# Gepetto/mpc-interface

Hardware: AMD Instinct MI355X
Metric: QP assemblies/sec (P,q,G,h), biped N=16 batched (higher is better)
Workload: dtype f64; 1 GPU; C2 biped LIPM N=16 no=36 nc=76, per-instance (A,B)/given/aim, K1 on chip; batch_per_gpu=4096, global_batch=4096, streams=2

## Files before the change

include/mpcasm.h:

```cpp
#ifndef MPCASM_H
#define MPCASM_H

#include <stddef.h>
#include <stdint.h>

#ifdef __cplusplus
extern "C" {
#endif

typedef enum mpcasm_status {
  MPCASM_OK = 0,
  MPCASM_ERR_ARG = -1,
  MPCASM_ERR_PLAN = -2,
  MPCASM_ERR_HIP = -3,
  MPCASM_ERR_NODEVICE = -4,
  MPCASM_ERR_LIMIT = -5
} mpcasm_status;

typedef struct mpcasm_plan mpcasm_plan;


int mpcasm_abi_version(void);
int mpcasm_device_count(void);
int mpcasm_last_hip(void);
const char* mpcasm_status_string(int status);
enum { MPCASM_OPT_PATH = 1, MPCASM_OPT_PHASE_MASK = 2, MPCASM_OPT_RESIDENT_PER_CU = 3, MPCASM_OPT_JIT = 4,
       MPCASM_OPT_P_DIRECT = 5, MPCASM_OPT_RESIDENT_GRID = 6 };
int mpcasm_set_option(int option, int value);
int mpcasm_plan_set_option(mpcasm_plan* plan, int option, int value);
int mpcasm_resident_lds_bytes(const int32_t* h_itab, size_t n_itab, const double* h_dtab, size_t n_dtab,
                              int64_t out[2]);
int mpcasm_jit_check(const int32_t* h_itab, size_t n_itab, const double* h_dtab, size_t n_dtab,
                     char* log, size_t log_capacity);

int mpcasm_plan_prepare(const mpcasm_plan* plan, int batch);
int mpcasm_jit_stats(int64_t out[3]);

int mpcasm_fill_su(const double* d_A, const double* d_B, double* d_S, double* d_U,
                   int batch, int N, int n, int m, int ltv, void* stream);

int mpcasm_plan_create(const int32_t* h_itab, size_t n_itab,
                       const double* h_dtab, size_t n_dtab,
                       mpcasm_plan** out_plan);
int mpcasm_plan_destroy(mpcasm_plan* plan);

int mpcasm_plan_sizes(const mpcasm_plan* plan, int64_t out[8]);

int mpcasm_plan_csc_sizes(const mpcasm_plan* plan, int64_t out[2]);
// ... 99 lines not shown
```

mpc-interface_amd/csrc/capi.hip:

```cpp
#include <hip/hip_runtime.h>
#include <stdint.h>
#include <stdlib.h>
#include <string.h>

#include <algorithm>
#include <cmath>
#include <mutex>
#include <new>
#include <string>
#include <vector>

#include "jit.h"
#include "kernels.h"

using namespace mpcasm;

namespace mpcasm {
int g_p_direct = 0;
extern int g_path;
extern int g_phase_mask;
extern int g_resident_per_cu, g_resident_grid;
}

struct mpcasm_plan {
// ... 1055 lines not shown
  if (option == MPCASM_OPT_P_DIRECT) {
    if (value < 0 || value > 2) return MPCASM_ERR_ARG;
    g_p_direct = value;
    return MPCASM_OK;
  }
  if (option == MPCASM_OPT_JIT) {
    if (value < 0 || value > 2) return MPCASM_ERR_ARG;
    g_jit = value;
    return MPCASM_OK;
  }
  if (option == MPCASM_OPT_RESIDENT_PER_CU) {
    if (value < 0 || value > 16) return MPCASM_ERR_ARG;
    g_resident_per_cu = value;
    return MPCASM_OK;
  }
  if (option == MPCASM_OPT_RESIDENT_GRID) {
    if (value < 0 || value > (1 << 20)) return MPCASM_ERR_ARG;
    g_resident_grid = value;
    return MPCASM_OK;
  }
  return MPCASM_ERR_ARG;
}

int mpcasm_plan_set_option(mpcasm_plan* plan, int option, int value) {
  if (!plan) return MPCASM_ERR_ARG;
  if (option == MPCASM_OPT_PATH && value >= -1 && value <= 4) plan->opt_path = value;
  else if (option == MPCASM_OPT_JIT && value >= -1 && value <= 2) plan->opt_jit = value;
  else if (option == MPCASM_OPT_RESIDENT_PER_CU && value >= -1 && value <= 16) plan->opt_per_cu = value;
  else if (option == MPCASM_OPT_RESIDENT_GRID && value >= -1 && value <= (1 << 20)) plan->opt_grid = value;
  else return MPCASM_ERR_ARG;
// ... 102 lines not shown
  PlanDev d;
  memset(&d, 0, sizeof d);
  plan_dev_from_tables(h_itab, &d);
  if (!d.rs_ok) return MPCASM_ERR_LIMIT;
  std::vector<char> code;
  std::string text;
  const int small = resident_p_direct_for(d, 1), large = resident_p_direct_for(d, 1 << 30);
  int out = MPCASM_OK;
  if (!jit_available()) {
    text = "libhiprtc.so could not be loaded";
    out = MPCASM_ERR_LIMIT;
  } else {
    for (int form : {small, large}) {
      if (form == large && small != large && out != MPCASM_OK) break;
      d.rs_p_direct = form;
      out = jit_code_for(jit_spec_header(d, h_itab), false, 0xBF, &code, &text) ? MPCASM_OK : MPCASM_ERR_HIP;
      if (small == large) break;
    }
  }
  if (log && log_capacity) {
    strncpy(log, text.c_str(), log_capacity - 1);
    log[log_capacity - 1] = 0;
  }
  return out;
}

int mpcasm_jit_stats(int64_t out[3]) {
  if (!out) return MPCASM_ERR_ARG;
  long v[3];
  jit_stats(v);
  out[0] = v[0];
  out[1] = v[1];
  out[2] = v[2];
  return MPCASM_OK;
}

int mpcasm_plan_prepare(const mpcasm_plan* plan, int batch) {
  if (!plan || batch < 0) return MPCASM_ERR_ARG;
  int current = -1;
// ... 460 lines not shown
```

mpc-interface_amd/csrc/jit.h:

```cpp
#pragma once
#include <hip/hip_runtime.h>
#include <stdint.h>

#include <string>
#include <vector>

#include "plan_dev.h"

namespace mpcasm {

extern int g_jit;
extern int g_phase_mask;

std::string jit_spec_header(const PlanDev& d, const int32_t* h_itab);
int jit_compile(const std::string& header, std::vector<char>* code, std::string* log,
                bool stamps = false, int phases = 0xBF);
const void* jit_kernel_for(const PlanDev& d, const int32_t* h_itab, int device, int batch,
                           size_t lds_bytes);
bool jit_code_for(const std::string& header, bool stamps, int phases, std::vector<char>* code,
                  std::string* log, bool distrust_disk = false);
bool jit_available();
void jit_stats(long out[3]);
void jit_forget(const void* itab);
int jit_launch(const void* kernel, const PlanDev& p, const SrcTable& src, const double* params,
               const double* given, double* P, double* q, double* G, double* h, int batch,
               int num_cus, int per_cu_limit, int grid_limit, void* work, hipStream_t stream, hipError_t* err);

}
```

mpc-interface_amd/csrc/jit.hip:

```cpp
#include <dlfcn.h>
#include <hip/hip_runtime.h>
#include <stdint.h>
#include <stdio.h>
#include <stdlib.h>
#include <string.h>

#include <sys/stat.h>
#include <sys/types.h>
#include <unistd.h>

#include <atomic>
#include <condition_variable>
#include <iterator>
#include <map>
#include <mutex>
#include <string>
#include <vector>

#include "jit.h"
#include "kernels.h"

namespace mpcasm {

int g_jit = 0;

namespace {

#include "jit_embed.inc"

constexpr int JIT_MIN_BATCH = 512;

struct Rtc {
  typedef struct _hiprtcProgram* Program;
  int (*create)(Program*, const char*, const char*, int, const char* const*, const char* const*);
  int (*compile)(Program, int, const char* const*);
  int (*log_size)(Program, size_t*);
  int (*get_log)(Program, char*);
  int (*code_size)(Program, size_t*);
  int (*get_code)(Program, char*);
// ... 20 lines not shown
    r.get_code = reinterpret_cast<decltype(r.get_code)>(sym("hiprtcGetCode"));
    r.destroy = reinterpret_cast<decltype(r.destroy)>(sym("hiprtcDestroyProgram"));
    r.ok = r.create && r.compile && r.log_size && r.get_log && r.code_size && r.get_code && r.destroy;
  });
  return r;
}

void append(std::string& s, const char* fmt, long long v) {
  char buf[96];
  snprintf(buf, sizeof buf, fmt, v);
  s += buf;
}

}

std::string jit_spec_header(const PlanDev& d, const int32_t* it) {
  std::string s = "// generated by libmpcasm (jit.hip) for one plan\n#pragma once\n"
                  "namespace mpcasm {\nnamespace spec {\nstruct PlanConst {\n";
#define MPCASM_X(f) append(s, "  static constexpr int " #f " = %lld;\n", (long long)d.f);
  MPCASM_PLAN_INT_FIELDS(MPCASM_X)
#undef MPCASM_X
  append(s, "  static constexpr unsigned rs_src16 = %lldu;\n};\n", (long long)d.rs_src16);
  const int jc = d.rs_jc <= 3 ? 3 : d.rs_jc <= 4 ? 4 : d.rs_jc <= 5 ? 5 : d.rs_jc <= 8 ? 8 : RS_JC_MAX;
  append(s, "constexpr int JC = %lld;\n", jc);
  append(s, "constexpr int NTRIP = %lld;\n", d.rs_ntrip);
  s += "constexpr int TRIPS[NTRIP + 1][8] = {\n";
  const int32_t* tr = it + d.off_rs_trip;
  for (int t = 0; t <= d.rs_ntrip; ++t) {
    s += "  {";
    for (int k = 0; k < RS_TRIP_WORDS; ++k) append(s, k ? ", %lld" : "%lld", tr[t * RS_TRIP_WORDS + k]);
    s += "},\n";
  }
  s += "};\nconstexpr int WTRIP[8][2] = {";
  const int32_t* wt = it + d.off_rs_wtrip;
  for (int w = 0; w < RS_WAVES; ++w) {
    append(s, "{%lld, ", wt[2 * w]);
    append(s, "%lld}, ", wt[2 * w + 1]);
  }
  s += "};\n}  // namespace spec\n}  // namespace mpcasm\n";
  return s;
}

int jit_compile(const std::string& header, std::vector<char>* code, std::string* log, bool stamps,
                int phases) {
  const Rtc& r = rtc();
  if (!r.ok) {
    if (log) *log = "libhiprtc.so could not be loaded";
    return MPCASM_ERR_LIMIT;
  }
  const char* headers[] = {header.c_str(), k_src_device_prims, k_src_plan_dev, k_src_plan_tables};
  const char* names[] = {"plan_spec.h", "device_prims.h", "plan_dev.h", "plan_tables.h"};
  Rtc::Program prog = nullptr;
// ... 110 lines not shown

struct JitKernel {
  hipModule_t module = nullptr;
  hipFunction_t fn = nullptr;
  int per_cu = 0;
  size_t lds = 0;
  bool failed = false;
  bool building = true;
};

std::mutex g_mutex;
std::condition_variable g_built;
std::map<std::pair<int, std::string>, JitKernel*> g_cache;
struct FastKey {
  const void* itab;
  int device, p_direct, phases;
  bool operator<(const FastKey& o) const {
    if (itab != o.itab) return itab < o.itab;
    if (device != o.device) return device < o.device;
    if (p_direct != o.p_direct) return p_direct < o.p_direct;
    return phases < o.phases;
  }
};
std::map<FastKey, JitKernel*> g_fast;

}

bool jit_code_for(const std::string& header, bool stamps, int phases, std::vector<char>* code,
                  std::string* log_out, bool distrust_disk) {
  const char* waves = getenv("MPCASM_JIT_WAVES_PER_EU");
  const std::string options = std::string(stamps ? "stamps " : "") + "phases " + std::to_string(phases) +
                              " waves " + (waves ? waves : "4") +
// ... 15 lines not shown
  }
  ++g_stat_compiled;
  if (getenv("MPCASM_JIT_VERBOSE")) fprintf(stderr, "mpcasm: jit: compiled (%zu bytes)\n", code->size());
  if (!path.empty()) disk_write(path, *code);
  return true;
}

namespace {
}

const void* jit_kernel_for(const PlanDev& d, const int32_t* h_itab, int device, int batch,
                           size_t lds_bytes) {
  if (t_jit == 2) return nullptr;
  const bool stamps = (g_phase_mask & 64) != 0;
  const int phases = stamps ? -1 : g_phase_mask;
  const FastKey fast{d.itab, stamps ? device + 4096 : device, d.rs_p_direct, phases};
  const bool may_build = t_jit == 1 || batch >= JIT_MIN_BATCH;
  JitKernel* slot = nullptr;
  bool mine = false;
  std::string header;
  {
    std::unique_lock<std::mutex> lock(g_mutex);
    auto found = g_fast.find(fast);
    if (found != g_fast.end()) {
      slot = found->second;
    } else if (may_build) {
      header = jit_spec_header(d, h_itab);
      JitKernel*& by_text = g_cache[std::make_pair(fast.device, header + "//" + std::to_string(phases))];
      if (by_text == nullptr) {
        by_text = new JitKernel();
        mine = true;
      }
      slot = by_text;
      g_fast[fast] = slot;
    } else {
      return nullptr;
    }
    if (!mine) {
      if (slot->building && !may_build) return nullptr;
      g_built.wait(lock, [&] { return !slot->building; });
    }
  }
// ... 93 lines not shown
```

mpc-interface_amd/csrc/plan_tables.h:

```cpp
#pragma once
#ifndef __HIPCC_RTC__
#include <stdint.h>
#endif

namespace mpcasm {

constexpr int32_t PLAN_MAGIC = 0x4D504341;
constexpr int32_t PLAN_VERSION = 30;

enum HeaderWord : int {
  H_MAGIC = 0,
  H_VERSION,
  H_NG,
  H_NO,
  H_NC,
  H_NPARAMS,
  H_NSRC,
  H_NBASE,
  H_NSEG,
  H_RTOT,
  H_NENT,
  H_NGTERM,
  H_NLIMIT,
  H_NLAX,
// ... 168 lines not shown
enum { GT_AOFF = 0, GT_BOFF, GT_NROWS, GT_WPARAM, GT_DOFF, GT_AIMPARAM, GT_FLAGS, GT_MASKA, GT_MASKB, GT_PAD, GT_WORDS = 10 };
enum { GT_FLAG_P = 1, GT_FLAG_HALF = 2, GT_FLAG_DIAG = 4 };

enum {
  LM_OUT0 = 0, LM_NROWS, LM_NAXES, LM_LAX0,
  LM_ARROW_P, LM_ARROW_ROWS, LM_CENTER_P, LM_CENTER_ROWS, LM_EXTREME_P, LM_EXTREME_ROWS,
  LM_PAD0, LM_PAD1, LM_WORDS = 12
};
enum { LX_ROWOFF = 0, LX_ROWS, LX_WORDS = 2 };

constexpr int MAX_SOURCES = 32;
constexpr int RS_NW = 4, RS_NT = 512, RS_WAVES = RS_NT / 64, RS_JC_MAX = 12, RS_TRIP_WORDS = 8;
constexpr int RS_BLOCKS_MAX = 255;
enum { LT_N = 0, LT_M, LT_HORIZON, LT_A, LT_B, LT_TA, LT_TB, LT_TP, RS_LTI_WORDS = 8 };
constexpr int RS_LTI_MAX = 4;
constexpr int RS_AXMAX = 4, RS_RR_WORDS = 16;
constexpr int RS_GDESC_PIECES = 6, RS_GDESC_THREADS = RS_NT - RS_NW * 64;
constexpr int RS_GFIX_NONE = 7;
constexpr int32_t RS_DST_ACC = 1 << 30;
enum { RT_A = 0, RT_B, RT_D, RT_W, RT_AIM, RT_WORD, RT_BI, RT_BJ };
enum { RT_SHORT = 5, RT_HALF = 6, RT_NOP = 7, RT_FIRST = 8, RT_LAST = 9, RT_LIVE = 10, RT_QMASK = 14,
       RT_TERM_END = 18 };
constexpr int RS_DIAG_MAX = 2;
enum { RR_VOFF = 0, RR_ARROW = 4, RR_CENTER = 8, RR_NAXES = 12, RR_EXTREME = 13, RR_PACKED = 14 };

}
```

mpc-interface_amd/csrc/resident.hip:

```cpp
#ifdef __HIPCC_RTC__
using __hip_internal::int32_t;
using __hip_internal::int64_t;
using __hip_internal::uint32_t;
using __hip_internal::uint64_t;
typedef unsigned long uintptr_t;
#else
#include <hip/hip_runtime.h>
#include <stdint.h>
#endif

#include "device_prims.h"
#include "plan_dev.h"
#ifdef MPCASM_SPEC
#include "plan_spec.h"
#endif
#ifndef __HIPCC_RTC__
#include "kernels.h"
#endif

namespace mpcasm {

#ifndef __HIPCC_RTC__
extern int g_phase_mask;
extern int g_resident_per_cu;
// ... 169 lines not shown
    int lk_ = s.lk, lx_ = s.lx;
    asm volatile("" : "+v"(lk_), "+v"(lx_));
    const int row = 4 * s.bi + lk_, col = 4 * s.bj + lx_;
    if (s.live && row < PC::no) {
      if (s.isq) {
        if (lx_ == 0) s.ql[row] = s.acc + s.dvec[ldp + row];
      } else if (col < PC::no) {
        const double val = s.acc + (row == col ? s.dvec[col] : 0.0);
        s.Pl[row * s.ldpl + col] = val;
        if (PC::rs_sym && s.bi != s.bj) s.Pl[col * s.ldpl + row] = val;
      }
    }
  }
}

template <int I, int N>
__device__ __forceinline__ void spec_trips(TripState& s) {
  if constexpr (I < N) {
    spec_trip<I>(s);
    __builtin_amdgcn_sched_barrier(0);
    spec_trips<I + 1, N>(s);
  }
}
template <int WAVE>
__device__ __forceinline__ void spec_wave_trips(TripState& s) {
  spec_trips<spec::WTRIP[WAVE][0], spec::WTRIP[WAVE][0] + spec::WTRIP[WAVE][1]>(s);
}
#endif

template <int JC, bool STAMPS, bool GEN, class PlanT>
// ... 42 lines not shown
  const int unit = p.rs_unit, nchunk = p.rs_nchunk;
  const int lx = lane & 3, lg = (lane >> 2) & 3, lk = lane >> 4;
  const unsigned ab_lds = (unsigned)(uintptr_t)(lds + L.ab);
  auto fetch_ab = [&](long inst, int slot) {
    for (int k = 0; k < p.rs_ab / 32; ++k) {
      const int2 m = abmeta[k * 64 + lane];
      const char* base = reinterpret_cast<const char* const*>(strm)[2 * m.x];
      const long long stride = reinterpret_cast<const long long*>(strm)[2 * m.x + 1];
      dma4(base + inst * stride + m.y,
           __builtin_amdgcn_readfirstlane(ab_lds + (unsigned)((slot * p.rs_ab + k * 32) * 8)));
    }
  };
  auto generate_sources = [&](int buf, int slot) {
    double* im = lds + L.img + buf * p.rs_img;
    const double* ab = lds + L.ab + slot * p.rs_ab;
    for (int g = 0; g < p.rs_nlti; ++g) {
      const int* rec = lti + g * RS_LTI_WORDS;
      const int n = __builtin_amdgcn_readfirstlane(rec[LT_N]), m = __builtin_amdgcn_readfirstlane(rec[LT_M]);
      const int N = __builtin_amdgcn_readfirstlane(rec[LT_HORIZON]), nn = n * n, nm = n * m;
      const double* Am = ab + __builtin_amdgcn_readfirstlane(rec[LT_A]);
      const double* Bm = ab + __builtin_amdgcn_readfirstlane(rec[LT_B]);
      double* TA = im + __builtin_amdgcn_readfirstlane(rec[LT_TA]);
      double* TB = im + __builtin_amdgcn_readfirstlane(rec[LT_TB]);
      double* TP = im + __builtin_amdgcn_readfirstlane(rec[LT_TP]);
      if (n <= 4 && n + m <= 4) {
        const int grp = lane >> 4, gi = lane & 3, gc = (lane >> 2) & 3;
        const bool live = gi < n && gc < n + m;
        double ar[4];
#pragma unroll
        for (int t = 0; t < 4; ++t) ar[t] = gi < n && t < n ? Am[gi * n + t] : 0.0;
        double x = !live ? 0.0 : (gc < m ? Bm[gi * m + gc] : Am[gi * n + (gc - m)]);
        double* out = gc < m ? TB + gi * m + gc : TA + gi * n + (gc - m);
        const int step = gc < m ? nm : nn;
        auto advance = [&]() {
          double y = ar[0] * quad_broadcast<0>(x);
          y = fma(ar[1], quad_broadcast<1>(x), y);
          y = fma(ar[2], quad_broadcast<2>(x), y);
          y = fma(ar[3], quad_broadcast<3>(x), y);
          x = y;
        };
        const int head = N < 4 ? N : 4;
        for (int d = 0; d < head; ++d) {
          if (live && grp == 0) out[d * step] = x;
          advance();
        }
        if (N > 4) {
          asm volatile("s_waitcnt lgkmcnt(0)" ::: "memory");
#pragma unroll
          for (int t = 0; t < 4; ++t) ar[t] = gi < n && t < n ? TA[3 * nn + gi * n + t] : 0.0;
          x = live ? out[grp * step] : 0.0;
          for (int d = grp + 4; d - grp < N; d += 4) {
            advance();
            if (live && d < N) out[d * step] = x;
          }
        }
        continue;
      }
      for (int e = lane; e < nn; e += 64) {
        const double v = Am[e];
        TA[e] = v;
        TP[e] = v;
      }
      for (int e = lane; e < nm; e += 64) TB[e] = Bm[e];
      asm volatile("s_waitcnt lgkmcnt(0)" ::: "memory");
      int have = 1;
      for (int s_ = 0; have < N; ++s_) {
        const double* Pw = TP + s_ * nn;
        const int cnt = have < N - have ? have : N - have;
        const int na = cnt * nn, nb = cnt * nm, total = na + nb + nn;
        for (int e = lane; e < total; e += 64) {
          const double* X;
// ... 7 lines not shown
            const int d = (e - na) / nm;
            r = (e - na) - d * nm;
            X = TB + d * nm, out = TB + (have + d) * nm, w = m;
          } else {
            r = e - na - nb;
            X = Pw, out = TP + (s_ + 1) * nn, w = n;
          }
          const int i = r / w, j = r - i * w;
          double acc = 0.0;
          for (int t = 0; t < n; ++t) acc = fma(Pw[i * n + t], X[t * w + j], acc);
          out[r] = acc;
        }
        asm volatile("s_waitcnt lgkmcnt(0)" ::: "memory");
        have += cnt;
      }
    }
  };
  const int run_over = (phases >> 10) & 7;
  const int run_shift = run_over ? run_over : ((long)batch >= 16L * gridDim.x && !(phases & 256) ? 2 : 0);
  const unsigned vblock = (phases & 8192) && gridDim.x % 8 == 0
                              ? (blockIdx.x % 8) * (gridDim.x / 8) + blockIdx.x / 8 : blockIdx.x;
  auto instance_at = [&](int n) -> long {
    return ((((long)(n >> run_shift) * gridDim.x + vblock)) << run_shift) + (n & ((1 << run_shift) - 1));
  };
  const bool gen = GEN && p.rs_nlti != 0;
  const int ct = tid - 64, CT = NT - 64;
#ifdef MPCASM_SPEC
  constexpr int ZK = 2;
#else
  constexpr int ZK = 0;
#endif
// ... 72 lines not shown
    for (int k = kfirst; k < nchunk; k += MW) {
      const int2 m = meta[k * 64 + lane];
      const char* base = reinterpret_cast<const char* const*>(strm)[2 * m.x];
      const long long stride = reinterpret_cast<const long long*>(strm)[2 * m.x + 1];
      if (settled && __all(stride == 0)) continue;
      const char* a = base + (m.x == p.nsrc ? ginst : inst) * stride + m.y;
      const unsigned dst = __builtin_amdgcn_readfirstlane(dst0 + (unsigned)(k * 64 * unit));
      if (unit == 16)
        dma16(a, dst);
      else
        dma4(a, dst);
    }
  };
  if (wave == 0) {
    constexpr int MK = 2;
    const int nab2 = p.rs_ab * 2, nmeta = nchunk * 64, nltw = p.rs_nlti * RS_LTI_WORDS;
    const int2* t_ab = reinterpret_cast<const int2*>(plan_itab + p.off_rs_abmeta);
    const int2* t_meta = reinterpret_cast<const int2*>(plan_itab + p.off_rs_inmeta);
    const int32_t* t_lti = plan_itab + p.off_rs_lti;
    int2 v_ab = int2{0, 0}, v_meta[MK];
    int v_lti = 0;
    if (lane < nab2) v_ab = t_ab[lane];
    if (lane < nltw) v_lti = t_lti[lane];
#pragma unroll
    for (int k = 0; k < MK; ++k) v_meta[k] = lane + k * 64 < nmeta ? t_meta[lane + k * 64] : int2{0, 0};
    if (prog_early) load_program();
    if (lane < nab2) abmeta[lane] = v_ab;
    for (int i = lane + 64; i < nab2; i += 64) abmeta[i] = t_ab[i];
    if (lane < nltw) lti[lane] = v_lti;
    for (int i = lane + 64; i < nltw; i += 64) lti[i] = t_lti[i];
#pragma unroll
    for (int k = 0; k < MK; ++k)
      if (lane + k * 64 < nmeta) meta[lane + k * 64] = v_meta[k];
    for (int i = lane + MK * 64; i < nmeta; i += 64) meta[i] = t_meta[i];
    for (int t = 0; t < p.nsrc + 3; ++t) {
      const int s = t - p.nsrc;
      const double* base = s < 0 ? src.ptr[t]
                                 : (s == 0 ? given : (s == 1 ? params : plan_dtab + p.doff_rs_const));
      const long long stride =
          s < 0 ? src.stride[t] : (s == 0 ? (long long)p.ng : (s == 1 ? (long long)p.nparams : 0));
      if (lane == 0) {
        reinterpret_cast<const double**>(strm)[2 * t] = base;
        reinterpret_cast<long long*>(strm)[2 * t + 1] = stride * (long long)sizeof(double);
      }
    }
    if (gen) {
      fetch_ab(instance_at(0), 0);
      if (instance_at(1) < batch) fetch_ab(instance_at(1), 1);
    }
    SETUP_STAMP(2)
    {
      const long inst = instance_at(0), ginst = gix != nullptr ? (long)gix[inst] : inst;
      for (int k = 0; k < nchunk; ++k) {
        const int2 m = meta[k * 64 + lane];
        const char* base = reinterpret_cast<const char* const*>(strm)[2 * m.x];
        const long long stride = reinterpret_cast<const long long*>(strm)[2 * m.x + 1];
        const char* a = base + (m.x == p.nsrc ? ginst : inst) * stride + m.y;
        const unsigned dst = __builtin_amdgcn_readfirstlane(img_lds + (unsigned)(k * 64 * unit));
        if (unit == 16)
          dma16(a, dst);
        else
          dma4(a, dst);
      }
    }
    SETUP_STAMP(0)
    lds_barrier();
    SETUP_STAMP(1)
    prepare_fetch();
    SETUP_STAMP(3)
    if (gen) {
      dma_wait_but(nchunk);
      SETUP_STAMP(4)
      generate_sources(0, 0);
    }
    if (!prog_early) load_program();
    SETUP_STAMP(5)
  } else {
    SETUP_STAMP(0)
    lds_barrier();
    SETUP_STAMP(1)
    prepare_fetch();
    SETUP_STAMP(2)
    load_program();
    typedef int i32x4 __attribute__((ext_vector_type(4)));
    typedef int i32x2 __attribute__((ext_vector_type(2)));
    typedef double f64x2 __attribute__((ext_vector_type(2)));
// ... 712 lines not shown
```

mpc-interface_amd/mpcasm/capi.py:

```python
import ctypes
import os

_HERE = os.path.dirname(os.path.abspath(__file__))
LIB_PATH = os.environ.get("MPCASM_LIB") or os.path.join(_HERE, "libmpcasm.so")

OK = 0
ERR_LIMIT = -5
OPT_PATH = 1
OPT_PHASE_MASK = 2
OPT_RESIDENT_PER_CU = 3
OPT_RESIDENT_GRID = 6
OPT_P_DIRECT = 5
OPT_JIT = 4
PHASE_DEFAULT = 0xBF
PHASE_STAMPS = 0x40
STATUS = {
    0: "MPCASM_OK",
    -1: "MPCASM_ERR_ARG",
    -2: "MPCASM_ERR_PLAN",
    -3: "MPCASM_ERR_HIP",
    -4: "MPCASM_ERR_NODEVICE",
    -5: "MPCASM_ERR_LIMIT",
}
QP_SOLVED, QP_MAX_ITER, QP_PRIMAL_INFEASIBLE, QP_DUAL_INFEASIBLE, QP_NON_CVX = 1, -2, -3, -4, -7
QP_STATUS = {
    1: "MPCASM_QP_SOLVED",
    -2: "MPCASM_QP_MAX_ITER",
# ... 13 lines not shown
    "mpcasm_abi_version": (ctypes.c_int, []),
    "mpcasm_device_count": (ctypes.c_int, []),
    "mpcasm_last_hip": (ctypes.c_int, []),
    "mpcasm_status_string": (ctypes.c_char_p, [ctypes.c_int]),
    "mpcasm_set_option": (ctypes.c_int, [ctypes.c_int, ctypes.c_int]),
    "mpcasm_fill_su": (ctypes.c_int, [_void_p, _void_p, _void_p, _void_p, ctypes.c_int,
                                      ctypes.c_int, ctypes.c_int, ctypes.c_int, ctypes.c_int,
                                      _void_p]),
    "mpcasm_plan_create": (ctypes.c_int, [_void_p, ctypes.c_size_t, _void_p, ctypes.c_size_t,
                                          ctypes.POINTER(_void_p)]),
    "mpcasm_plan_destroy": (ctypes.c_int, [_void_p]),
    "mpcasm_resident_lds_bytes": (ctypes.c_int, [_void_p, ctypes.c_size_t, _void_p, ctypes.c_size_t,
                                                 ctypes.POINTER(ctypes.c_int64)]),
    "mpcasm_jit_check": (ctypes.c_int, [_void_p, ctypes.c_size_t, _void_p, ctypes.c_size_t,
                                        ctypes.c_char_p, ctypes.c_size_t]),
    "mpcasm_plan_sizes": (ctypes.c_int, [_void_p, ctypes.POINTER(ctypes.c_int64)]),
    "mpcasm_plan_csc_sizes": (ctypes.c_int, [_void_p, ctypes.POINTER(ctypes.c_int64)]),
    "mpcasm_plan_set_option": (ctypes.c_int, [_void_p, ctypes.c_int, ctypes.c_int]),
    "mpcasm_assemble_indexed": (ctypes.c_int, [_void_p, ctypes.POINTER(_void_p),
                                               ctypes.POINTER(ctypes.c_int64), _void_p, _void_p, _void_p,
                                               _void_p, _void_p, _void_p, _void_p, _void_p, ctypes.c_int,
                                               _void_p]),
    "mpcasm_plan_last_kernel": (ctypes.c_int, [_void_p]),
    "mpcasm_plan_prepare": (ctypes.c_int, [_void_p, ctypes.c_int]),
    "mpcasm_jit_stats": (ctypes.c_int, [ctypes.POINTER(ctypes.c_int64)]),
    "mpcasm_workspace_bytes": (ctypes.c_int, [_void_p, ctypes.c_int,
                                              ctypes.POINTER(ctypes.c_size_t)]),
    "mpcasm_assemble": (ctypes.c_int, [_void_p, ctypes.POINTER(_void_p),
                                       ctypes.POINTER(ctypes.c_int64), _void_p, _void_p, _void_p,
                                       _void_p, _void_p, _void_p, _void_p, ctypes.c_int, _void_p]),
# ... 89 lines not shown
```

mpc-interface_amd/mpcasm/plan.py:

```python
import collections
import hashlib
from types import SimpleNamespace

import numpy as np
import scipy.sparse as sp

PLAN_MAGIC = 0x4D504341
PLAN_VERSION = 30

_H = {name: i for i, name in enumerate([
    "MAGIC", "VERSION", "NG", "NO", "NC", "NPARAMS", "NSRC", "NBASE", "NSEG", "RTOT", "NENT",
    "NGTERM", "NLIMIT", "NLAX", "PMROWS", "PM_NENT", "LDV",
    "OFF_SEG", "OFF_COLSEG", "OFF_ROWPTR", "OFF_ENTBASE", "OFF_ENTK", "OFF_GTERM", "OFF_LIMIT",
    "OFF_LAX", "OFF_ROWLIMIT", "OFF_PM_ROWPTR", "OFF_PM_ENTBASE", "OFF_PM_ENTK",
    "DOFF_ENTCOEF", "DOFF_PM_ENTCOEF", "NITAB", "NDTAB",
    "FUSED_OK", "ARENA_TOTAL", "OFF_ARENA", "NFD", "OFF_FD_IDX", "OFF_FD_PTR", "NOPS", "OFF_OP",
    "NCOEF", "DOFF_COEFPOOL",
    "RS_OK", "RS_JC", "RS_SYM", "RS_NTRIP", "OFF_RS_SRC", "OFF_RS_GIDX", "OFF_RS_DST",
    "DOFF_RS_COEF", "OFF_RS_TRIP", "OFF_RS_WTRIP", "RS_NSPLIT", "OFF_RS_SPLIT",
    "OFF_RS_RR", "RS_UNIT", "RS_NCHUNK", "OFF_RS_INMETA", "RS_IMG", "RS_IMG_GIVEN",
    "RS_IMG_PARAMS", "DOFF_RS_CONST", "DOFF_DIAGCOEF", "NDIAGCOEF", "RS_NLTI", "OFF_RS_LTI",
    "RS_IMG_DMA", "RS_AB", "OFF_RS_ABMETA", "RR_PACKED", "OFF_RS_DPAR", "DOFF_RS_DCOEF",
    "RS_NGDESC", "OFF_RS_GDESC", "PM_NFD", "OFF_PM_MAP", "OFF_PM_FDPTR", "OFF_PM_OP", "PM_NOPS",
    "DOFF_PM_POOL", "PM_NPOOL", "RS_NZBLK", "OFF_RS_ZBLK", "RS_GSINGLE",
# ... 8 lines not shown
    "SW_OK", "SW_N", "SW_M", "SW_HORIZON", "SW_SRC_A", "SW_SRC_B", "SW_NAXES", "OFF_SW_AXIS", "SW_NTERM",
    "OFF_SW_TERM", "SW_NLIM", "OFF_SW_LIM", "OFF_SW_COL", "SW_DOFF_CVEC", "SW_NCVEC",
    "OFF_SW_CPTR", "OFF_SW_CENT", "SW_NCENT", "OFF_SW_GPTR", "OFF_SW_GENT", "SW_NGENT",
    "OFF_RS_PROG", "T_SCAN_FUSED",
])}
H_WORDS = 160
assert len(_H) <= H_WORDS
RS_NW, RS_NT = 4, 512
RS_WAVES = RS_NT // 64
RS_BLOCKS_MAX = 255
RS_LTI_WORDS, RS_LTI_MAX = 8, 4
RS_JC_MAX = 12
RS_TRIP_WORDS = 8
TRIP_COST, TRIP_STEP_COST, TERM_COST, TRIP_Q_COST, PACK_COST, G_PIECE_COST = 200, 30, 60, 60, 250, 500
G_DESC_PIECE_COST = 330
TABLES_COST, STREAM_WAVE_COST, FETCH_CHUNK_COST = 3300, 500, 350
import os as _os
if _os.environ.get("MPCASM_TRIP_COSTS"):
    _c = [int(x) for x in _os.environ["MPCASM_TRIP_COSTS"].split(",")]
    TRIP_COST, TRIP_STEP_COST, TERM_COST, TRIP_Q_COST, PACK_COST, G_PIECE_COST = _c[:6]
    G_DESC_PIECE_COST = G_PIECE_COST
    if len(_c) > 6:
        TABLES_COST, STREAM_WAVE_COST, FETCH_CHUNK_COST = _c[6:9]
RT_A, RT_B, RT_D, RT_W, RT_AIM, RT_WORD, RT_BI, RT_BJ = range(8)
RT_SHORT, RT_HALF, RT_NOP, RT_FIRST, RT_LAST, RT_LIVE, RT_QMASK, RT_TERM_END = 5, 6, 7, 8, 9, 10, 14, 18
RS_DIAG_MAX = 2
RS_AXMAX = 4
RS_DST_ACC = 1 << 30
RS_GDESC_PIECES, RS_GDESC_THREADS = 6, 256
RS_GFIX_NONE = 7
RS_COMPACT_FROM_BYTES = 65536
RS_RR_WORDS = 16
SEG_WORDS, GT_WORDS, LM_WORDS, LX_WORDS = 8, 10, 12, 2
FUSED_MAX_OPS = 1 << 18
FUSED_MAX_ARENA = 1 << 14
SEG_GATHER, SEG_IDENTITY = 0, 1
GT_FLAG_P, GT_FLAG_HALF, GT_FLAG_DIAG = 1, 2, 4
MAX_SOURCES = 32
# ... 762 lines not shown
        word = trip[RT_WORD]
        if not word & 31:
            return 0
        return (TRIP_COST + (TRIP_STEP_COST if (word >> RT_SHORT) & 1 else 4 * TRIP_STEP_COST)
                + (TERM_COST + (TRIP_Q_COST if (word >> RT_QMASK) & 15 else 0)
                   if (word >> RT_TERM_END) & 1 else 0))

    cost = [PACK_COST + sum(trip_cost(trip) for trip in lst) for lst in pack_trips]
    stream_threads = NT - NW * 64
    pieces = nc_rows * max(no // 2, 1)
    by_descriptor = no % 2 == 0 and pieces <= RS_GDESC_PIECES * RS_GDESC_THREADS

    loads = []
    for w in range(RS_WAVES):
        if w < NW:
            gen = TABLES_COST if image["groups"] and w == NW - 1 else 0
            loads.append((FETCH_CHUNK_COST * len(range(w, image["nchunk"], NW)) + gen, w))
        else:
            first = (w - NW) * 64
            own = len(range(first, pieces, stream_threads))
            loads.append(((G_DESC_PIECE_COST if by_descriptor else G_PIECE_COST) * own + STREAM_WAVE_COST, w))
    heapq.heapify(loads)
    wave_packs = [[] for _ in range(RS_WAVES)]
    for k in sorted(range(len(pack_trips)), key=lambda k: -cost[k]):
        load, w = heapq.heappop(loads)
        wave_packs[w].append(k)
        heapq.heappush(loads, (load + cost[k], w))
    trips, wtrip = [], np.zeros(RS_WAVES * 2, dtype=np.int32)
    for w in range(RS_WAVES):
        wtrip[2 * w] = len(trips)
        for k in wave_packs[w]:
# ... 999 lines not shown
```

Measured before the change: 167.6 million assemblies/s.

## Specialize JIT resident kernel fetch addressing with compile-time run segments

Compresses each chunk's per-lane fetch metadata into a few arithmetic runs (stream, base byte, step, period) and emits them as constexpr tables in the JIT header. The specialized kernel then computes fetch addresses directly and issues the first A/B and image DMAs without loading meta tables from global memory first. LTI generator records also become compile-time constants. The wave cost model lowers the table-generation cost for small-state groups. This adds template recursion and code size, and the host planner's cost change may move work onto different waves.

```diff
diff --git a/include/mpcasm.h b/include/mpcasm.h
--- a/include/mpcasm.h
+++ b/include/mpcasm.h
@@ -25,13 +25,15 @@
 int mpcasm_last_hip(void);
 const char* mpcasm_status_string(int status);
 enum { MPCASM_OPT_PATH = 1, MPCASM_OPT_PHASE_MASK = 2, MPCASM_OPT_RESIDENT_PER_CU = 3, MPCASM_OPT_JIT = 4,
-       MPCASM_OPT_P_DIRECT = 5, MPCASM_OPT_RESIDENT_GRID = 6 };
+       MPCASM_OPT_P_DIRECT = 5, MPCASM_OPT_RESIDENT_GRID = 6, MPCASM_OPT_JIT_FETCH_RUNS = 7 };
 int mpcasm_set_option(int option, int value);
 int mpcasm_plan_set_option(mpcasm_plan* plan, int option, int value);
 int mpcasm_resident_lds_bytes(const int32_t* h_itab, size_t n_itab, const double* h_dtab, size_t n_dtab,
                               int64_t out[2]);
 int mpcasm_jit_check(const int32_t* h_itab, size_t n_itab, const double* h_dtab, size_t n_dtab,
                      char* log, size_t log_capacity);
+int mpcasm_fetch_segments(const int32_t* h_itab, size_t n_itab, const double* h_dtab, size_t n_dtab,
+                          int limit, int32_t* out, size_t capacity, int64_t* n_words);
 
 int mpcasm_plan_prepare(const mpcasm_plan* plan, int batch);
 int mpcasm_jit_stats(int64_t out[3]);
diff --git a/mpc-interface_amd/csrc/capi.hip b/mpc-interface_amd/csrc/capi.hip
--- a/mpc-interface_amd/csrc/capi.hip
+++ b/mpc-interface_amd/csrc/capi.hip
@@ -1093,6 +1093,11 @@
     g_resident_per_cu = value;
     return MPCASM_OK;
   }
+  if (option == MPCASM_OPT_JIT_FETCH_RUNS) {
+    if (value < 0 || value > FS_MAX) return MPCASM_ERR_ARG;
+    g_jit_fetch_runs = value;
+    return MPCASM_OK;
+  }
   if (option == MPCASM_OPT_RESIDENT_GRID) {
     if (value < 0 || value > (1 << 20)) return MPCASM_ERR_ARG;
     g_resident_grid = value;
@@ -1225,7 +1230,7 @@
     for (int form : {small, large}) {
       if (form == large && small != large && out != MPCASM_OK) break;
       d.rs_p_direct = form;
-      out = jit_code_for(jit_spec_header(d, h_itab), false, 0xBF, &code, &text) ? MPCASM_OK : MPCASM_ERR_HIP;
+      out = jit_code_for(jit_spec_header(d, h_itab, g_jit_fetch_runs), false, 0xBF, &code, &text) ? MPCASM_OK : MPCASM_ERR_HIP;
       if (small == large) break;
     }
   }
@@ -1234,6 +1239,22 @@
     log[log_capacity - 1] = 0;
   }
   return out;
+}
+
+int mpcasm_fetch_segments(const int32_t* h_itab, size_t n_itab, const double* h_dtab, size_t n_dtab,
+                          int limit, int32_t* out, size_t capacity, int64_t* n_words) {
+  if (!h_itab || (n_dtab && !h_dtab) || !n_words || (capacity && !out) || limit < 0) return MPCASM_ERR_ARG;
+  const int rc = validate_plan(h_itab, h_dtab, n_itab, n_dtab);
+  if (rc != MPCASM_OK) return rc;
+  PlanDev d;
+  memset(&d, 0, sizeof d);
+  plan_dev_from_tables(h_itab, &d);
+  if (!d.rs_ok) return MPCASM_ERR_LIMIT;
+  const std::vector<int32_t> words = jit_fetch_plan(d, h_itab, limit);
+  *n_words = (int64_t)words.size();
+  if (words.size() > capacity) return MPCASM_ERR_LIMIT;
+  if (!words.empty()) memcpy(out, words.data(), words.size() * sizeof(int32_t));
+  return MPCASM_OK;
 }
 
 int mpcasm_jit_stats(int64_t out[3]) {
diff --git a/mpc-interface_amd/csrc/jit.h b/mpc-interface_amd/csrc/jit.h
--- a/mpc-interface_amd/csrc/jit.h
+++ b/mpc-interface_amd/csrc/jit.h
@@ -10,9 +10,11 @@
 namespace mpcasm {
 
 extern int g_jit;
+extern int g_jit_fetch_runs;
 extern int g_phase_mask;
 
-std::string jit_spec_header(const PlanDev& d, const int32_t* h_itab);
+std::string jit_spec_header(const PlanDev& d, const int32_t* h_itab, int seg_limit = FS_MAX);
+std::vector<int32_t> jit_fetch_plan(const PlanDev& d, const int32_t* h_itab, int seg_limit);
 int jit_compile(const std::string& header, std::vector<char>* code, std::string* log,
                 bool stamps = false, int phases = 0xBF);
 const void* jit_kernel_for(const PlanDev& d, const int32_t* h_itab, int device, int batch,
diff --git a/mpc-interface_amd/csrc/jit.hip b/mpc-interface_amd/csrc/jit.hip
--- a/mpc-interface_amd/csrc/jit.hip
+++ b/mpc-interface_amd/csrc/jit.hip
@@ -23,6 +23,7 @@
 namespace mpcasm {
 
 int g_jit = 0;
+int g_jit_fetch_runs = FS_MAX;
 
 namespace {
 
@@ -73,7 +74,43 @@
 
 }
 
-std::string jit_spec_header(const PlanDev& d, const int32_t* it) {
+std::vector<int32_t> jit_fetch_segments(const int32_t* meta, int lanes) {
+  std::vector<int32_t> out;
+  for (int i = 0; i < lanes;) {
+    const int stream = meta[2 * i], byte0 = meta[2 * i + 1];
+    const int step = i + 1 < lanes && meta[2 * (i + 1)] == stream ? meta[2 * (i + 1) + 1] - byte0 : 0;
+    int best = 0, best_period = 0;
+    for (int period : {0, 4, 2, 1}) {
+      int n = 0;
+      while (i + n < lanes && meta[2 * (i + n)] == stream &&
+             meta[2 * (i + n) + 1] == byte0 + (period ? n % period : n) * (period == 1 ? 0 : step))
+        ++n;
+      if (n > best) best = n, best_period = period;
+    }
+    const int period = best_period && best_period < best ? best_period : best;
+    out.insert(out.end(), {i, best, stream, byte0, best > 1 && period > 1 ? step : 0, period});
+    i += best;
+  }
+  return out;
+}
+
+std::vector<int32_t> jit_fetch_plan(const PlanDev& d, const int32_t* it, int limit) {
+  std::vector<int32_t> out;
+  if (limit > FS_MAX) limit = FS_MAX;
+  for (int kind = 0; kind < 2; ++kind) {
+    const int chunks = kind == 0 ? d.rs_ab / 32 : d.rs_nchunk;
+    const int32_t* meta = it + (kind == 0 ? d.off_rs_abmeta : d.off_rs_inmeta);
+    for (int k = 0; k < chunks; ++k) {
+      std::vector<int32_t> segs = jit_fetch_segments(meta + k * 128, 64);
+      if ((int)segs.size() > limit * FS_WORDS || (kind == 1 && k >= 32)) segs.clear();
+      out.insert(out.end(), {kind, k, (int32_t)(segs.size() / FS_WORDS)});
+      out.insert(out.end(), segs.begin(), segs.end());
+    }
+  }
+  return out;
+}
+
+std::string jit_spec_header(const PlanDev& d, const int32_t* it, int seg_limit) {
   std::string s = "// generated by libmpcasm (jit.hip) for one plan\n#pragma once\n"
                   "namespace mpcasm {\nnamespace spec {\nstruct PlanConst {\n";
 #define MPCASM_X(f) append(s, "  static constexpr int " #f " = %lld;\n", (long long)d.f);
@@ -95,6 +132,39 @@
   for (int w = 0; w < RS_WAVES; ++w) {
     append(s, "{%lld, ", wt[2 * w]);
     append(s, "%lld}, ", wt[2 * w + 1]);
+  }
+  s += "};\n";
+  const std::vector<int32_t> fetch = jit_fetch_plan(d, it, seg_limit);
+  for (int kind = 0; kind < 2; ++kind) {
+    const int chunks = kind == 0 ? d.rs_ab / 32 : d.rs_nchunk;
+    const char* name = kind == 0 ? "AB" : "IMG";
+    std::string counts, table;
+    long long on_table = 0;
+    for (size_t at = 0; at < fetch.size(); at += 3 + fetch[at + 2] * FS_WORDS) {
+      if (fetch[at] != kind) continue;
+      const int n = fetch[at + 2];
+      if (n == 0 && fetch[at + 1] < 32) on_table |= 1ll << fetch[at + 1];
+      append(counts, "%lld, ", n);
+      table += "  {";
+      for (int g = 0; g < FS_MAX; ++g) {
+        table += "{";
+        for (int w = 0; w < FS_WORDS; ++w) append(table, w ? ", %lld" : "%lld", g < n ? fetch[at + 3 + g * FS_WORDS + w] : 0);
+        table += "}, ";
+      }
+      table += "},\n";
+    }
+    if (chunks == 0) counts = "0", table = "  {},\n";
+    s += std::string("constexpr int FSEG_") + name + "_N[] = {" + counts + "};\n";
+    s += std::string("constexpr int FSEG_") + name + "[][8][6] = {\n" + table + "};\n";
+    s += std::string("constexpr unsigned FSEG_") + name + "_TABLE = ";
+    append(s, "%lldu;\n", on_table);
+  }
+  s += "constexpr int LTI[4][8] = {\n";
+  for (int g = 0; g < RS_LTI_MAX; ++g) {
+    s += "  {";
+    for (int w = 0; w < RS_LTI_WORDS; ++w)
+      append(s, w ? ", %lld" : "%lld", g < d.rs_nlti ? it[d.off_rs_lti + g * RS_LTI_WORDS + w] : 0);
+    s += "},\n";
   }
   s += "};\n}  // namespace spec\n}  // namespace mpcasm\n";
   return s;
@@ -235,8 +305,9 @@
 std::map<std::pair<int, std::string>, JitKernel*> g_cache;
 struct FastKey {
   const void* itab;
-  int device, p_direct, phases;
+  int device, p_direct, phases, fetch_runs;
   bool operator<(const FastKey& o) const {
+    if (fetch_runs != o.fetch_runs) return fetch_runs < o.fetch_runs;
     if (itab != o.itab) return itab < o.itab;
     if (device != o.device) return device < o.device;
     if (p_direct != o.p_direct) return p_direct < o.p_direct;
@@ -282,7 +353,7 @@
   if (t_jit == 2) return nullptr;
   const bool stamps = (g_phase_mask & 64) != 0;
   const int phases = stamps ? -1 : g_phase_mask;
-  const FastKey fast{d.itab, stamps ? device + 4096 : device, d.rs_p_direct, phases};
+  const FastKey fast{d.itab, stamps ? device + 4096 : device, d.rs_p_direct, phases, g_jit_fetch_runs};
   const bool may_build = t_jit == 1 || batch >= JIT_MIN_BATCH;
   JitKernel* slot = nullptr;
   bool mine = false;
@@ -293,7 +364,7 @@
     if (found != g_fast.end()) {
       slot = found->second;
     } else if (may_build) {
-      header = jit_spec_header(d, h_itab);
+      header = jit_spec_header(d, h_itab, fast.fetch_runs);
       JitKernel*& by_text = g_cache[std::make_pair(fast.device, header + "//" + std::to_string(phases))];
       if (by_text == nullptr) {
         by_text = new JitKernel();
diff --git a/mpc-interface_amd/csrc/plan_tables.h b/mpc-interface_amd/csrc/plan_tables.h
--- a/mpc-interface_amd/csrc/plan_tables.h
+++ b/mpc-interface_amd/csrc/plan_tables.h
@@ -206,6 +206,8 @@
 constexpr int RS_BLOCKS_MAX = 255;
 enum { LT_N = 0, LT_M, LT_HORIZON, LT_A, LT_B, LT_TA, LT_TB, LT_TP, RS_LTI_WORDS = 8 };
 constexpr int RS_LTI_MAX = 4;
+enum { FS_FIRST = 0, FS_LANES, FS_STREAM, FS_BYTE, FS_STEP, FS_PERIOD, FS_WORDS = 6 };
+constexpr int FS_MAX = 8;
 constexpr int RS_AXMAX = 4, RS_RR_WORDS = 16;
 constexpr int RS_GDESC_PIECES = 6, RS_GDESC_THREADS = RS_NT - RS_NW * 64;
 constexpr int RS_GFIX_NONE = 7;
diff --git a/mpc-interface_amd/csrc/resident.hip b/mpc-interface_amd/csrc/resident.hip
--- a/mpc-interface_amd/csrc/resident.hip
+++ b/mpc-interface_amd/csrc/resident.hip
@@ -207,6 +207,107 @@
   }
 }
 
+struct LaneSrc {
+  const char* base;
+  long long stride;
+  bool isg;
+  int2 entry;
+};
+static_assert(FS_MAX == 8 && FS_WORDS == 6 && RS_LTI_MAX == 4 && RS_LTI_WORDS == 8, "plan_spec.h, as jit.hip writes it");
+template <bool AB, int K>
+constexpr int spec_fetch_runs() {
+  if constexpr (AB)
+    return K < spec::PlanConst::rs_ab / 32 ? spec::FSEG_AB_N[K] : 0;
+  else
+    return K < spec::PlanConst::rs_nchunk ? spec::FSEG_IMG_N[K] : 0;
+}
+template <bool AB, int K, int S>
+__device__ __forceinline__ void spec_lane_run(LaneSrc& out, int lane, const SrcTable& src, const double* params,
+                                              const double* given, const double* plan_dtab) {
+  using PC = spec::PlanConst;
+  if constexpr (S < spec_fetch_runs<AB, K>()) {
+    constexpr int first = AB ? spec::FSEG_AB[K][S][FS_FIRST] : spec::FSEG_IMG[K][S][FS_FIRST];
+    constexpr int lanes = AB ? spec::FSEG_AB[K][S][FS_LANES] : spec::FSEG_IMG[K][S][FS_LANES];
+    constexpr int stream = AB ? spec::FSEG_AB[K][S][FS_STREAM] : spec::FSEG_IMG[K][S][FS_STREAM];
+    constexpr int byte0 = AB ? spec::FSEG_AB[K][S][FS_BYTE] : spec::FSEG_IMG[K][S][FS_BYTE];
+    constexpr int step = AB ? spec::FSEG_AB[K][S][FS_STEP] : spec::FSEG_IMG[K][S][FS_STEP];
+    constexpr int period = AB ? spec::FSEG_AB[K][S][FS_PERIOD] : spec::FSEG_IMG[K][S][FS_PERIOD];
+    static_assert(period >= lanes || (period & (period - 1)) == 0, "a periodic run repeats every 1, 2 or 4 lanes");
+    const char* base;
+    long long stride;
+    if constexpr (stream < PC::nsrc) {
+      base = reinterpret_cast<const char*>(src.ptr[stream]);
+      stride = src.stride[stream] * (long long)sizeof(double);
+    } else if constexpr (stream == PC::nsrc) {
+      base = reinterpret_cast<const char*>(given);
+      stride = (long long)PC::ng * (long long)sizeof(double);
+    } else if constexpr (stream == PC::nsrc + 1) {
+      base = reinterpret_cast<const char*>(params);
+      stride = (long long)PC::nparams * (long long)sizeof(double);
+    } else {
+      base = reinterpret_cast<const char*>(plan_dtab + PC::doff_rs_const);
+      stride = 0;
+    }
+    const int rel = lane - first;
+    const int off = byte0 + (period < lanes ? rel & (period - 1) : rel) * step;
+    if (S == 0 || lane >= first) {
+      out.base = base + off;
+      out.stride = stride;
+      out.isg = stream == PC::nsrc;
+      out.entry = int2{stream, off};
+    }
+    spec_lane_run<AB, K, S + 1>(out, lane, src, params, given, plan_dtab);
+  }
+}
+template <bool AB, int K>
+__device__ __forceinline__ LaneSrc spec_lane_src(int lane, const SrcTable& src, const double* params,
+                                                 const double* given, const double* plan_dtab) {
+  LaneSrc out{nullptr, 0, false, int2{0, 0}};
+  spec_lane_run<AB, K, 0>(out, lane, src, params, given, plan_dtab);
+  return out;
+}
+template <bool AB, int K>
+__device__ __forceinline__ void spec_write_table(int2* table, int lane, const SrcTable& src, const double* params,
+                                                 const double* given, const double* plan_dtab) {
+  if constexpr (K < (AB ? spec::PlanConst::rs_ab / 32 : spec::PlanConst::rs_nchunk)) {
+    table[K * 64 + lane] = spec_lane_src<AB, K>(lane, src, params, given, plan_dtab).entry;
+    spec_write_table<AB, K + 1>(table, lane, src, params, given, plan_dtab);
+  }
+}
+template <int K>
+__device__ __forceinline__ void spec_first_ab(int lane, long inst0, long inst1, bool two, unsigned ab_lds,
+                                              const SrcTable& src, const double* params, const double* given,
+                                              const double* plan_dtab) {
+  using PC = spec::PlanConst;
+  if constexpr (K < PC::rs_ab / 32) {
+    const LaneSrc m = spec_lane_src<true, K>(lane, src, params, given, plan_dtab);
+    dma4(m.base + inst0 * m.stride, ab_lds + (unsigned)(K * 32 * 8));
+    if (two) dma4(m.base + inst1 * m.stride, ab_lds + (unsigned)((PC::rs_ab + K * 32) * 8));
+    spec_first_ab<K + 1>(lane, inst0, inst1, two, ab_lds, src, params, given, plan_dtab);
+  }
+}
+template <int K>
+__device__ __forceinline__ void spec_first_image(int lane, long inst, long ginst, unsigned img_lds, const SrcTable& src,
+                                                 const double* params, const double* given, const double* plan_dtab) {
+  using PC = spec::PlanConst;
+  if constexpr (K < PC::rs_nchunk && K < 32) {
+    if constexpr (spec_fetch_runs<false, K>() != 0) {
+      const LaneSrc m = spec_lane_src<false, K>(lane, src, params, given, plan_dtab);
+      const char* a = m.base + (m.isg ? ginst : inst) * m.stride;
+      if constexpr (PC::rs_unit == 16)
+        dma16(a, img_lds + (unsigned)(K * 64 * 16));
+      else
+        dma4(a, img_lds + (unsigned)(K * 64 * 4));
+    }
+    spec_first_image<K + 1>(lane, inst, ginst, img_lds, src, params, given, plan_dtab);
+  }
+}
+constexpr bool spec_ab_by_runs() {
+  for (int k = 0; k < spec::PlanConst::rs_ab / 32; ++k)
+    if (spec::FSEG_AB_N[k] == 0) return false;
+  return true;
+}
+
 template <int I, int N>
 __device__ __forceinline__ void spec_trips(TripState& s) {
   if constexpr (I < N) {
@@ -279,17 +380,20 @@
   auto generate_sources = [&](int buf, int slot) {
     double* im = lds + L.img + buf * p.rs_img;
     const double* ab = lds + L.ab + slot * p.rs_ab;
-    for (int g = 0; g < p.rs_nlti; ++g) {
-      const int* rec = lti + g * RS_LTI_WORDS;
-      const int n = __builtin_amdgcn_readfirstlane(rec[LT_N]), m = __builtin_amdgcn_readfirstlane(rec[LT_M]);
-      const int N = __builtin_amdgcn_readfirstlane(rec[LT_HORIZON]), nn = n * n, nm = n * m;
-      const double* Am = ab + __builtin_amdgcn_readfirstlane(rec[LT_A]);
-      const double* Bm = ab + __builtin_amdgcn_readfirstlane(rec[LT_B]);
-      double* TA = im + __builtin_amdgcn_readfirstlane(rec[LT_TA]);
-      double* TB = im + __builtin_amdgcn_readfirstlane(rec[LT_TB]);
-      double* TP = im + __builtin_amdgcn_readfirstlane(rec[LT_TP]);
+    auto generate = [&](auto word) __attribute__((always_inline)) {
+      const int n = word(LT_N), m = word(LT_M);
+      const int N = word(LT_HORIZON), nn = n * n, nm = n * m;
+      const double* Am = ab + word(LT_A);
+      const double* Bm = ab + word(LT_B);
+      double* TA = im + word(LT_TA);
+      double* TB = im + word(LT_TB);
+      double* TP = im + word(LT_TP);
       if (n <= 4 && n + m <= 4) {
-        const int grp = lane >> 4, gi = lane & 3, gc = (lane >> 2) & 3;
+        int lane_ = lane;
+#ifdef MPCASM_SPEC
+        asm volatile("" : "+v"(lane_));
+#endif
+        const int grp = lane_ >> 4, gi = lane_ & 3, gc = (lane_ >> 2) & 3;
         const bool live = gi < n && gc < n + m;
         double ar[4];
 #pragma unroll
@@ -319,7 +423,7 @@
             if (live && d < N) out[d * step] = x;
           }
         }
-        continue;
+        return;
       }
       for (int e = lane; e < nn; e += 64) {
         const double v = Am[e];
@@ -357,7 +461,18 @@
         asm volatile("s_waitcnt lgkmcnt(0)" ::: "memory");
         have += cnt;
       }
-    }
+    };
+#ifdef MPCASM_SPEC
+    if constexpr (PlanT::rs_nlti > 0) generate([](int k) { return spec::LTI[0][k]; });
+    if constexpr (PlanT::rs_nlti > 1) generate([](int k) { return spec::LTI[1][k]; });
+    if constexpr (PlanT::rs_nlti > 2) generate([](int k) { return spec::LTI[2][k]; });
+    if constexpr (PlanT::rs_nlti > 3) generate([](int k) { return spec::LTI[3][k]; });
+#else
+    for (int g = 0; g < p.rs_nlti; ++g) {
+      const int* rec = lti + g * RS_LTI_WORDS;
+      generate([&](int k) { return __builtin_amdgcn_readfirstlane(rec[k]); });
+    }
+#endif
   };
   const int run_over = (phases >> 10) & 7;
   const int run_shift = run_over ? run_over : ((long)batch >= 16L * gridDim.x && !(phases & 256) ? 2 : 0);
@@ -460,25 +575,61 @@
   };
   if (wave == 0) {
     constexpr int MK = 2;
-    const int nab2 = p.rs_ab * 2, nmeta = nchunk * 64, nltw = p.rs_nlti * RS_LTI_WORDS;
+#ifdef MPCASM_SPEC
+    constexpr int nltw = 0;
+#else
+    const int nltw = p.rs_nlti * RS_LTI_WORDS;
+#endif
+    const int nab2 = p.rs_ab * 2, nmeta = nchunk * 64;
     const int2* t_ab = reinterpret_cast<const int2*>(plan_itab + p.off_rs_abmeta);
     const int2* t_meta = reinterpret_cast<const int2*>(plan_itab + p.off_rs_inmeta);
     const int32_t* t_lti = plan_itab + p.off_rs_lti;
     int2 v_ab = int2{0, 0}, v_meta[MK];
     int v_lti = 0;
-    if (lane < nab2) v_ab = t_ab[lane];
+#ifdef MPCASM_SPEC
+    constexpr bool ab_runs = spec_ab_by_runs();
+    constexpr unsigned on_table = spec::FSEG_IMG_TABLE;
+    constexpr bool img_runs = on_table == 0 && PlanT::rs_nchunk <= 32;
+    constexpr int img_late = __builtin_popcount(on_table) + (PlanT::rs_nchunk > 32 ? PlanT::rs_nchunk - 32 : 0);
+    const int ab_later = ab_runs ? nchunk : img_late;
+    if (gen && ab_runs) {
+      const long i1 = instance_at(1);
+      spec_first_ab<0>(lane, instance_at(0), i1, i1 < batch, __builtin_amdgcn_readfirstlane(ab_lds), src, params,
+                       given, plan_dtab);
+    }
+    if (ab_runs) SETUP_STAMP(2)
+    {
+      const long inst = instance_at(0), ginst = gix != nullptr ? (long)gix[inst] : inst;
+      spec_first_image<0>(lane, inst, ginst, __builtin_amdgcn_readfirstlane(img_lds), src, params, given, plan_dtab);
+    }
+#else
+    constexpr bool ab_runs = false, img_runs = false;
+    constexpr unsigned on_table = ~0u;
+    const int ab_later = nchunk;
+#endif
+    if (!ab_runs && lane < nab2) v_ab = t_ab[lane];
     if (lane < nltw) v_lti = t_lti[lane];
-#pragma unroll
-    for (int k = 0; k < MK; ++k) v_meta[k] = lane + k * 64 < nmeta ? t_meta[lane + k * 64] : int2{0, 0};
+    if (!img_runs) {
+#pragma unroll
+      for (int k = 0; k < MK; ++k) v_meta[k] = lane + k * 64 < nmeta ? t_meta[lane + k * 64] : int2{0, 0};
+    }
     if (prog_early) load_program();
-    if (lane < nab2) abmeta[lane] = v_ab;
-    for (int i = lane + 64; i < nab2; i += 64) abmeta[i] = t_ab[i];
+    if (!ab_runs) {
+      if (lane < nab2) abmeta[lane] = v_ab;
+      for (int i = lane + 64; i < nab2; i += 64) abmeta[i] = t_ab[i];
+    }
     if (lane < nltw) lti[lane] = v_lti;
     for (int i = lane + 64; i < nltw; i += 64) lti[i] = t_lti[i];
-#pragma unroll
-    for (int k = 0; k < MK; ++k)
-      if (lane + k * 64 < nmeta) meta[lane + k * 64] = v_meta[k];
-    for (int i = lane + MK * 64; i < nmeta; i += 64) meta[i] = t_meta[i];
+    if (!img_runs) {
+#pragma unroll
+      for (int k = 0; k < MK; ++k)
+        if (lane + k * 64 < nmeta) meta[lane + k * 64] = v_meta[k];
+      for (int i = lane + MK * 64; i < nmeta; i += 64) meta[i] = t_meta[i];
+    }
+#ifdef MPCASM_SPEC
+    if constexpr (ab_runs) spec_write_table<true, 0>(abmeta, lane, src, params, given, plan_dtab);
+    if constexpr (img_runs) spec_write_table<false, 0>(meta, lane, src, params, given, plan_dtab);
+#endif
     for (int t = 0; t < p.nsrc + 3; ++t) {
       const int s = t - p.nsrc;
       const double* base = s < 0 ? src.ptr[t]
@@ -490,14 +641,15 @@
         reinterpret_cast<long long*>(strm)[2 * t + 1] = stride * (long long)sizeof(double);
       }
     }
-    if (gen) {
+    if (gen && !ab_runs) {
       fetch_ab(instance_at(0), 0);
       if (instance_at(1) < batch) fetch_ab(instance_at(1), 1);
     }
-    SETUP_STAMP(2)
-    {
+    if (!ab_runs) SETUP_STAMP(2)
+    if (!img_runs) {
       const long inst = instance_at(0), ginst = gix != nullptr ? (long)gix[inst] : inst;
       for (int k = 0; k < nchunk; ++k) {
+        if (k < 32 && !((on_table >> k) & 1)) continue;
         const int2 m = meta[k * 64 + lane];
         const char* base = reinterpret_cast<const char* const*>(strm)[2 * m.x];
         const long long stride = reinterpret_cast<const long long*>(strm)[2 * m.x + 1];
@@ -515,7 +667,7 @@
     prepare_fetch();
     SETUP_STAMP(3)
     if (gen) {
-      dma_wait_but(nchunk);
+      dma_wait_but(ab_later);
       SETUP_STAMP(4)
       generate_sources(0, 0);
     }
diff --git a/mpc-interface_amd/mpcasm/capi.py b/mpc-interface_amd/mpcasm/capi.py
--- a/mpc-interface_amd/mpcasm/capi.py
+++ b/mpc-interface_amd/mpcasm/capi.py
@@ -11,6 +11,7 @@
 OPT_RESIDENT_PER_CU = 3
 OPT_RESIDENT_GRID = 6
 OPT_P_DIRECT = 5
+OPT_JIT_FETCH_RUNS = 7
 OPT_JIT = 4
 PHASE_DEFAULT = 0xBF
 PHASE_STAMPS = 0x40
@@ -54,6 +55,8 @@
                                                  ctypes.POINTER(ctypes.c_int64)]),
     "mpcasm_jit_check": (ctypes.c_int, [_void_p, ctypes.c_size_t, _void_p, ctypes.c_size_t,
                                         ctypes.c_char_p, ctypes.c_size_t]),
+    "mpcasm_fetch_segments": (ctypes.c_int, [_void_p, ctypes.c_size_t, _void_p, ctypes.c_size_t, ctypes.c_int,
+                                             _void_p, ctypes.c_size_t, ctypes.POINTER(ctypes.c_int64)]),
     "mpcasm_plan_sizes": (ctypes.c_int, [_void_p, ctypes.POINTER(ctypes.c_int64)]),
     "mpcasm_plan_csc_sizes": (ctypes.c_int, [_void_p, ctypes.POINTER(ctypes.c_int64)]),
     "mpcasm_plan_set_option": (ctypes.c_int, [_void_p, ctypes.c_int, ctypes.c_int]),
diff --git a/mpc-interface_amd/mpcasm/plan.py b/mpc-interface_amd/mpcasm/plan.py
--- a/mpc-interface_amd/mpcasm/plan.py
+++ b/mpc-interface_amd/mpcasm/plan.py
@@ -46,7 +46,8 @@
 RS_TRIP_WORDS = 8
 TRIP_COST, TRIP_STEP_COST, TERM_COST, TRIP_Q_COST, PACK_COST, G_PIECE_COST = 200, 30, 60, 60, 250, 500
 G_DESC_PIECE_COST = 330
-TABLES_COST, STREAM_WAVE_COST, FETCH_CHUNK_COST = 3300, 500, 350
+TABLES_COST, STREAM_WAVE_COST, FETCH_CHUNK_COST = 2200, 500, 350
+TABLES_COST_GENERAL = 3300
 import os as _os
 if _os.environ.get("MPCASM_TRIP_COSTS"):
     _c = [int(x) for x in _os.environ["MPCASM_TRIP_COSTS"].split(",")]
@@ -54,6 +55,7 @@
     G_DESC_PIECE_COST = G_PIECE_COST
     if len(_c) > 6:
         TABLES_COST, STREAM_WAVE_COST, FETCH_CHUNK_COST = _c[6:9]
+        TABLES_COST_GENERAL = TABLES_COST
 RT_A, RT_B, RT_D, RT_W, RT_AIM, RT_WORD, RT_BI, RT_BJ = range(8)
 RT_SHORT, RT_HALF, RT_NOP, RT_FIRST, RT_LAST, RT_LIVE, RT_QMASK, RT_TERM_END = 5, 6, 7, 8, 9, 10, 14, 18
 RS_DIAG_MAX = 2
@@ -846,7 +848,8 @@
     loads = []
     for w in range(RS_WAVES):
         if w < NW:
-            gen = TABLES_COST if image["groups"] and w == NW - 1 else 0
+            small = all(g["n"] <= 4 and g["n"] + g["m"] <= 4 for g in image["groups"])
+            gen = (TABLES_COST if small else TABLES_COST_GENERAL) if image["groups"] and w == NW - 1 else 0
             loads.append((FETCH_CHUNK_COST * len(range(w, image["nchunk"], NW)) + gen, w))
         else:
             first = (w - NW) * 64
```

New measurement: 178.7 million assemblies/s, median of 6. 1.07x the previous value.
